# Tonanguyxiro/FastBN

Hardware: AMD Instinct MI355X
Metric: JT test-cases/sec (ALARM, Munin) + PC-stable CI-tests/sec, 1/2/4/8 GPU (higher is better)
Workload: dtype f64

## Files before the change

fastbn_amd/api.py:

```python
import atexit
import ctypes as C
import weakref
import os

import numpy as np

_HERE = os.path.dirname(os.path.abspath(__file__))
LIB_PATH = os.environ.get("FBN_LIB_PATH") or os.path.join(_HERE, "libfastbn.so")

_vp, _i32, _i64, _dbl, _cstr = C.c_void_p, C.c_int32, C.c_int64, C.c_double, C.c_char_p
_pp = C.POINTER(C.c_void_p)

_SIGS = {
    "fbn_version": [_vp, _vp],
    "fbn_device_count": [_vp],
    "fbn_network_load_xmlbif": [_cstr, _pp],
    "fbn_network_create": [C.c_int, _vp, _vp, _vp, _vp, _vp, _pp],
    "fbn_network_node_counts": [_vp, C.c_int, _vp, _vp, _vp, _vp],
    "fbn_network_num_nodes": [_vp, _vp],
    "fbn_network_dims": [_vp, _vp],
    "fbn_network_name": [_vp, C.c_int, C.c_char_p, C.c_int],
    "fbn_network_destroy": [_vp],
    "fbn_evidence_load_libsvm": [_cstr, C.c_int, _vp, _vp, _i64, _vp],
    "fbn_dataset_load_csv": [_cstr, _pp],
# ... 6 lines not shown
    "fbn_dataset_columns": [_vp, _vp],
    "fbn_dataset_var_name": [_vp, C.c_int, C.c_char_p, C.c_int],
    "fbn_dataset_destroy": [_vp],
    "fbn_jt_plan_create": [_vp, C.c_int, _pp],
    "fbn_jt_plan_info_get": [_vp, _vp],
    "fbn_jt_plan_dump": [_vp, _cstr, _cstr],
    "fbn_jt_run": [_vp, _vp, _i64, _vp, _vp, _vp],
    "fbn_jt_run_device": [_vp, _vp, _i64, _vp, _vp, _vp],
    "fbn_jt_evidence_validate": [_vp, _vp, _i64, _vp],
    "fbn_jt_set_evidence_check": [_vp, C.c_int],
    "fbn_jt_set_kernel_timing": [_vp, C.c_int],
    "fbn_jt_score": [_vp, _vp, _vp, _i64, _vp, _vp],
    "fbn_jt_set_output_layout": [_vp, C.c_int],
    "fbn_jt_score_terms_device": [_vp, _vp, _vp, _i64, _vp, _vp],
    "fbn_jt_last_kernel_ms": [_vp, _vp],
    "fbn_jt_stream_schedule": [_vp, _vp, C.c_int64, _vp, C.c_int64, _vp, _vp],
    "fbn_jt_set_waves_per_cu": [_vp, C.c_int],
    "fbn_jt_set_variant": [_vp, C.c_int],
    "fbn_jt_debug_op_cycles": [_vp, C.c_int, _vp],
    "fbn_jt_kernel_source": [_vp, C.c_char_p, C.c_int64, _vp],
    "fbn_jt_kernel_cache_path": [_vp, C.c_char_p, C.c_int64],
    "fbn_jt_kernel_options": [C.c_char_p, C.c_int64],
    "fbn_jt_kernel_build": [_vp],
    "fbn_jt_debug_force_fixup": [_vp, C.c_int],
    "fbn_jt_debug_flagged_blocks": [_vp, _vp],
    "fbn_jt_set_exact": [_vp, C.c_int],
    "fbn_jt_plan_destroy": [_vp],
    "fbn_ci_dataset_upload": [_vp, C.c_int, _i64, _vp, C.c_int, _pp],
    "fbn_ci_dataset_from_device": [_vp, C.c_int, _i64, _vp, C.c_int, _pp],
    "fbn_ci_set_kernel_timing": [_vp, C.c_int],
    "fbn_ci_run": [_vp, _vp, _i64, C.c_int, _dbl, _vp, _vp, _vp, _vp, _vp],
    "fbn_ci_counts": [_vp, C.c_int, C.c_int, _vp, C.c_int, _vp, _i64, _vp],
    "fbn_ci_last_kernel_ms": [_vp, _vp],
    "fbn_ci_decision_margin": [_vp, _vp, _vp, C.c_int],
    "fbn_ci_debug_counts": [_vp, _vp, _i64, C.c_int, _vp, _i64],
    "fbn_pc_decision_margin": [_vp, _vp, _vp],
    "fbn_ci_ctx_destroy": [_vp],
    "fbn_pc_stable": [_vp, _dbl, C.c_int, C.c_int, _pp],
    "fbn_pc_num_levels": [_vp, _vp],
    "fbn_pc_level_tests": [_vp, _vp],
    "fbn_pc_level_launched": [_vp, _vp],
    "fbn_pc_num_edges": [_vp, _vp],
    "fbn_pc_edges": [_vp, _vp],
    "fbn_pc_sepsets": [_vp, _vp, _i64, _vp],
    "fbn_pc_timing": [_vp, _vp, _vp],
    "fbn_pc_path": [_vp, _vp],
# ... 316 lines not shown
        buf = C.create_string_buffer(4096)
        lib.fbn_jt_kernel_cache_path(self._h, buf, 4096)
        return buf.value.decode()

    def debug_force_fixup(self, enable):
        lib.fbn_jt_debug_force_fixup(self._h, int(enable))

    def debug_flagged_blocks(self):
        n = C.c_int64()
        lib.fbn_jt_debug_flagged_blocks(self._h, C.byref(n))
        return n.value

    def set_exact(self, exact):
        lib.fbn_jt_set_exact(self._h, -1 if exact is None else int(bool(exact)))

    def build_kernel(self):
        lib.fbn_jt_kernel_build(self._h)
        return self.kernel_cache_path()

    def refresh_info(self):
        info = _PlanInfo()
        lib.fbn_jt_plan_info_get(self._h, C.byref(info))
        self.info = {k: getattr(info, k) for k, _ in _PlanInfo._fields_}
        return self.info

    def set_variant(self, v):
        lib.fbn_jt_set_variant(self._h, v)

    def infer(self, evidence, marginals=True):
        ev = np.ascontiguousarray(evidence, dtype=np.int8)
        n = ev.shape[0]
        labels = np.zeros(n, np.int32)
        marg = np.zeros((n, self.info["sum_dom"]), np.float64) if marginals else None
        lib.fbn_jt_run(self._h, _p(ev), n, _p(labels), _p(marg), None)
        return labels, marg

    def run_device(self, d_evidence_ptr, ncases, d_labels_ptr, d_marg_ptr, stream_ptr=None):
        lib.fbn_jt_run_device(self._h, d_evidence_ptr, ncases, d_labels_ptr, d_marg_ptr, stream_ptr)

    def validate_device(self, d_evidence_ptr, ncases, stream_ptr=None):
        lib.fbn_jt_evidence_validate(self._h, d_evidence_ptr, ncases, stream_ptr)

    def set_kernel_timing(self, enable):
        lib.fbn_jt_set_kernel_timing(self._h, int(bool(enable)))

    def set_evidence_check(self, enable):
# ... 389 lines not shown
```

fastbn_amd/csrc/capi.hip:

```cpp
#include <hip/hip_runtime.h>
#include <hipcub/hipcub.hpp>
#include <rocblas/rocblas.h>
#include <dlfcn.h>
#include <chrono>

#include <algorithm>
#include <cmath>
#include <cstdio>
#include <cstring>
#include <functional>
#include <memory>
#include <new>
#include <string>

#include "fbn_internal.h"
#include "sample_model.h"
#include "pc_internal.h"
#include "ci_chisq.h"
#include "pc_small.h"
#include "param_counts.h"

extern "C" hipError_t fbn_jt_launch(const JtOp *ops, int nops, const int32_t *aux, const double *initv,
                                    const uint64_t *dig, const int8_t *evid, int V, long long ncases, int SD,
                                    double *marg, int32_t *labels, double *ws, int32_t *wsi, long long NE, int nc,
// ... 764 lines not shown
    int rc = fbn::GenerateJTKernel(p->host, src, &we, iv, nullptr, JtFast(p), p->out_layout == 1);
    if (rc) return rc;
    if (len) *len = (int64_t)src.size() + 1;
    if (buf && cap > 0) {
        const size_t n = std::min<size_t>((size_t)cap - 1, src.size());
        memcpy(buf, src.data(), n);
        buf[n] = 0;
    }
    return FBN_OK;
}

int fbn_jt_kernel_cache_path(const fbn_jt_plan *p, char *buf, int64_t cap) {
    if (!p || !buf || cap <= 0) return SetError(FBN_ERR_ARG, "bad argument");
    if (!p->gen_eligible) return SetError(FBN_ERR_ARG, "plan not eligible for codegen");
    std::string src;
    std::vector<double> iv;
    int64_t we = 0;
    int rc = fbn::GenerateJTKernel(p->host, src, &we, iv, nullptr, JtFast(p), p->out_layout == 1);
    if (rc) return rc;
    snprintf(buf, (size_t)cap, "%s", fbn::JitCachePath(src).c_str());
    return FBN_OK;
}

int fbn_jt_set_exact(fbn_jt_plan *p, int exact) {
    if (!p || exact < -1 || exact > 1) return SetError(FBN_ERR_ARG, "exact must be -1 (auto), 0 (fast) or 1 (exact)");
    p->exact = exact;
    return FBN_OK;
}

int fbn_jt_debug_force_fixup(fbn_jt_plan *p, int enable) {
    if (!p) return SetError(FBN_ERR_ARG, "null pointer");
    p->force_fixup = enable != 0;
    return FBN_OK;
}

int fbn_jt_debug_flagged_blocks(fbn_jt_plan *p, int64_t *count) {
    if (!p || !count) return SetError(FBN_ERR_ARG, "null pointer");
    *count = 0;
    if (p->last_nblk <= 0 || !p->flags.p) return FBN_OK;
    std::vector<int> h((size_t)p->last_nblk);
    FBN_HIP(hipDeviceSynchronize());
    FBN_HIP(hipMemcpy(h.data(), p->flags.p, h.size() * 4, hipMemcpyDeviceToHost));
    for (int f : h) *count += f != 0;
    return FBN_OK;
}

// ... 2035 lines not shown
```

fastbn_amd/csrc/fbn_internal.h:

```cpp
#ifndef FBN_INTERNAL_H
#define FBN_INTERNAL_H

#include <cstdint>
#include <map>
#include <set>
#include <string>
#include <vector>

#include "../../include/fastbn.h"
#include "jt_program.h"

namespace fbn {

int SetError(int code, const char *fmt, ...);

struct Network {
    std::vector<std::string> names;
    std::vector<int> dom;
    std::vector<std::vector<int>> given;
    std::vector<std::vector<int>> parents_asc;
    std::vector<std::vector<int64_t>> counts;
    std::vector<std::vector<int64_t>> totals;
    int n() const { return (int)dom.size(); }
    double Prob(int v, int q, const int *parent_vals_asc) const;
// ... 81 lines not shown
    int64_t store_rows = 0;
    int64_t scratch_row = 0;
    int64_t scratch_rows = 0;
    int num_cliques = 0;
    int sum_dom = 0;
};
int CompileJTProgramV(const JTPlanHost &plan, JTProgramV &prog);

struct JTProgramT {
    std::vector<JtTPass> passes;
    std::vector<int32_t> tab;
    std::vector<double> initv;
    int64_t scr_row = 0;
    int64_t red_row = 0;
    int64_t store_rows = 0;
    int64_t lds_bytes = 0;
    int64_t entry_visits = 0;
    int num_cliques = 0, sum_dom = 0;
    int waves = 1;
};
int CompileJTProgramT(const JTPlanHost &plan, JTProgramT &prog, int lds_budget);

bool JTCodegenEligible(const JTPlanHost &plan, int64_t *entry_ops);
int GenerateJTKernel(const JTPlanHost &plan, std::string &src, int64_t *wave_entries, std::vector<double> &initv,
                     int64_t *lds_bytes = nullptr, bool fast = false, bool var_major = false);

}

struct fbn_network {
    fbn::Network net;
};
struct fbn_dataset {
    fbn::Dataset ds;
};

#endif
```

fastbn_amd/csrc/jt_codegen.cpp:

```cpp
#include <algorithm>
#include <map>
#include <cstdio>
#include <cstdlib>
#include <functional>
#include <sstream>
#include <string>

#include "fbn_internal.h"

namespace fbn {

namespace {

int LocOfT(const Table &t, int v) {
    for (size_t i = 0; i < t.vars.size(); ++i)
        if (t.vars[i] == v) return (int)i;
    return -1;
}

std::string Lit(double x) {
    char b[64];
    snprintf(b, sizeof b, "%.17g", x);
    std::string s = b;
    if (s.find_first_of(".eEn") == std::string::npos) s += ".0";
// ... 4 lines not shown

bool JTCodegenEligible(const JTPlanHost &plan, int64_t *entry_ops) {
    int64_t tmax = 0, ops = 0;
    for (const auto &t : plan.cliques) {
        tmax = std::max<int64_t>(tmax, t.size());
        ops += t.size() * (4 + (int64_t)t.vars.size());
    }
    if (entry_ops) *entry_ops = ops;
    for (int d : plan.dom)
        if (d > 32) return false;
    return tmax <= 256 && ops <= 40000;
}

namespace {

constexpr int kDefaultMerge = 1;

class JTGen {
  public:
    JTGen(const JTPlanHost &p, bool fast_order, bool var_major) : plan(p), fast(fast_order), vmajor(var_major) {}
    int Run(std::string &src, int64_t *wave_entries, std::vector<double> &initv);
    int64_t lds_rows = 0;
    int64_t pool_rows = 0;
    bool iv_lds = false;

  private:
    const JTPlanHost &plan;
    const bool fast;
    const bool vmajor;
    std::ostringstream o;
    std::vector<int> okw_word, okw_pos, out_off;
    std::vector<int64_t> sep_row, init_off;
    std::vector<std::vector<int>> cand;
    std::vector<int> home;
    std::vector<int> msep;
    std::vector<int> mclq;
    void ChooseMarginalSources(const std::vector<int> &pre);
    void MargTerms(int v, const std::vector<std::vector<std::string>> &terms);
    int nobs = 0;
    bool profile = false;
    int merge = 0;
    int64_t init_batch = 16;
    bool in_merged = false;
    int min_waves = 1;
    bool marg_v2 = true, marg_pair = true;
    std::vector<std::vector<std::string>> col_loc, dis_loc;
    std::vector<bool> md_reg;
    std::vector<bool> leaf_rc, col_store;
    void LoadCol(const std::string &name, int s) {
        if (!leaf_rc[s]) return Load(name, s);
        const int c = plan.sep_down[s];
        const int64_t Ts = plan.seps[s].size(), Q = plan.cliques[c].size() / Ts;
        for (int64_t j = 0; j < Ts; ++j) o << "        double " << name << s << "_" << j << ";\n";
        o << "        { // recompute the Collect message of leaf clique " << c << "\n";
        const std::string P = "r" + name;
        InitProd(P, c, {}, -1, "");
        for (int64_t j = 0; j < Ts; ++j) {
            std::vector<std::string> terms;
            for (int64_t q = 0; q < Q; ++q) terms.push_back(N(P, c, q * Ts + j));
            o << "        " << name << s << "_" << j << " = " << TreeSum(terms) << ";\n";
        }
        o << "        }\n";
    }
    void PlaceMessages(const std::vector<int> &post, const std::vector<int> &pre, int64_t budget);
    std::string B(int k) const {
        return profile ? "        FBN_OP_BOUNDARY(); FBN_STAMP(" + std::to_string(k) + ");\n" : "        FBN_OP_BOUNDARY();\n";
    }

    std::string R(int c) const {
        std::vector<unsigned> m(nobs, 0u);
        for (int v : plan.cliques[c].vars) m[v / 32] |= 1u << (v % 32);
        std::ostringstream t;
        t << "(" << plan.cliques[c].vars.size();
        for (int k = 0; k < nobs; ++k)
            if (m[k]) t << " - __builtin_popcount(obs" << k << " & " << m[k] << "u)";
        t << ")";
        return t.str();
    }
    std::string observed(int v) const {
        std::ostringstream t;
        t << "((obs" << v / 32 << " >> " << v % 32 << ") & 1u)";
        return t.str();
    }
    int child(int s) const { return plan.sep_down[s]; }
    int64_t SepIndex(const Table &t, const Table &sp, int64_t e) const {
        int64_t r = e, idx = 0;
        for (size_t j = 0; j < t.vars.size(); ++j) {
// ... 352 lines not shown

void JTGen::ChooseMarginalSources(const std::vector<int> &pre) {
    const int mode = getenv("FBN_JT_MARG_SRC") ? atoi(getenv("FBN_JT_MARG_SRC")) : 0;
    if (mode == 0 || getenv("FBN_JT_NO_SEPMARG")) return;
    const int nc = (int)plan.cliques.size(), ns = (int)plan.seps.size(), V = (int)plan.dom.size();
    std::vector<int> pi(nc);
    for (int k = 0; k < nc; ++k) pi[pre[k]] = k;
    for (int v = 0; v < V; ++v) {
        int best_t = -1, bc = -1, bs = -1;
        int64_t best_sz = 0;
        auto consider = [&](int t, int64_t sz, int c, int sp) {
            const bool better = best_t < 0 || (mode == 1 ? t > best_t : t < best_t) || (t == best_t && sz < best_sz);
            if (better) best_t = t, best_sz = sz, bc = c, bs = sp;
        };
        for (int c : cand[v]) consider(pi[c], plan.cliques[c].size(), c, -1);
        for (int sp = 0; sp < ns; ++sp)
            for (int u : plan.seps[sp].vars)
                if (u == v) consider(pi[plan.sep_up[sp]], plan.seps[sp].size(), -1, sp);
        if (bs >= 0) msep[v] = bs;
        else msep[v] = -1, mclq[v] = bc;
    }
}

void JTGen::PlaceMessages(const std::vector<int> &post, const std::vector<int> &pre, int64_t budget) {
    const int nc = (int)plan.cliques.size(), ns = (int)plan.seps.size();
    auto tsize = [&](int c) { return plan.cliques[c].size(); };
    std::vector<int> pi(nc), qi(nc);
    for (int k = 0; k < nc; ++k) qi[post[k]] = k, pi[pre[k]] = k;
    md_reg.assign(ns, false);
    for (int c : pre)
        if (!plan.clique_down[c].empty()) {
            const int q = pre[pi[c] + 1], s = plan.clique_up[q];
            int64_t mk = 0;
            for (int s2 : plan.clique_down[q]) mk = std::max<int64_t>(mk, plan.seps[s2].size());
            md_reg[s] = tsize(q) + plan.seps[s].size() + mk <= budget;
        }
    const bool no_leaf_rc = !getenv("FBN_JT_LEAF_RC") || atoi(getenv("FBN_JT_LEAF_RC")) == 0;
    leaf_rc.assign(ns, false);
    col_store.assign(ns, true);
    for (int s = 0; s < ns; ++s) {
        const int c = plan.sep_down[s], p = plan.sep_up[s];
        if (!fast || no_leaf_rc || !plan.clique_down[c].empty() || tsize(c) > 64) continue;
        leaf_rc[s] = true;
        col_store[s] = !(qi[p] > 0 && post[qi[p] - 1] == c);
    }
    struct Item {
        int s;
        bool dist;
        int a, b;
        int64_t n;
    };
    std::vector<Item> items;
    for (int s = 0; s < ns; ++s) {
        const int c = plan.sep_down[s], p = plan.sep_up[s];
        if (!leaf_rc[s]) items.push_back({s, false, qi[c], nc + pi[p], plan.seps[s].size()});
        else if (col_store[s]) items.push_back({s, false, qi[c], qi[p], plan.seps[s].size()});
        if (!md_reg[s]) items.push_back({s, true, nc + pi[p], nc + pi[c], plan.seps[s].size()});
    }
    const int64_t per_wave = 160 * 1024 / 4 / 8;
    int64_t ivn = 0;
    for (const auto &t : plan.cliques) ivn += t.size();
    int64_t cap = std::max<int64_t>(0, (per_wave - lds_rows * 64 - (iv_lds ? ivn : 0)) / 64);
    if (const char *e = getenv("FBN_JT_LDS_POOL")) cap = std::min<int64_t>(cap, std::max(0, atoi(e)));
    std::vector<int> order(items.size());
    for (size_t i = 0; i < items.size(); ++i) order[i] = (int)i;
    std::stable_sort(order.begin(), order.end(), [&](int x, int y) {
        return items[x].b - items[x].a < items[y].b - items[y].a;
    });
    std::vector<int64_t> use(2 * nc + 1, 0);
    std::vector<bool> in_lds(items.size(), false);
    for (int i : order) {
        const Item &it = items[i];
        if (it.n > cap) continue;
        int64_t mx = 0;
        for (int t = it.a; t <= it.b; ++t) mx = std::max(mx, use[t]);
        if (mx + it.n > cap) continue;
        for (int t = it.a; t <= it.b; ++t) use[t] += it.n;
        in_lds[i] = true;
    }
    std::vector<int> byst;
    for (size_t i = 0; i < items.size(); ++i)
        if (in_lds[i]) byst.push_back((int)i);
    std::stable_sort(byst.begin(), byst.end(), [&](int x, int y) { return items[x].a < items[y].a; });
    std::vector<std::vector<int64_t>> rows_of(items.size());
    std::vector<int64_t> free_rows;
    for (int64_t r = cap - 1; r >= 0; --r) free_rows.push_back(r);
    std::vector<int> active;
    pool_rows = 0;
    for (int i : byst) {
        const Item &it = items[i];
        for (size_t k = 0; k < active.size();) {
            if (items[active[k]].b < it.a) {
                for (int64_t r : rows_of[active[k]]) free_rows.push_back(r);
                std::sort(free_rows.rbegin(), free_rows.rend());
                active.erase(active.begin() + k);
            } else {
                ++k;
            }
        }
        for (int64_t j = 0; j < it.n; ++j) {
            rows_of[i].push_back(free_rows.back());
            pool_rows = std::max<int64_t>(pool_rows, free_rows.back() + 1);
            free_rows.pop_back();
        }
        active.push_back(i);
    }
    col_loc.assign(ns, {});
    dis_loc.assign(ns, {});
    sep_row.assign(ns, -1);
    int64_t grow = 0;
    for (size_t i = 0; i < items.size(); ++i) {
        const Item &it = items[i];
        auto &loc = it.dist ? dis_loc[it.s] : col_loc[it.s];
        loc.assign(it.n, std::string());
        if (in_lds[i]) {
            for (int64_t j = 0; j < it.n; ++j) loc[j] = "LP(" + std::to_string(rows_of[i][j]) + ")";
            continue;
        }
        if (sep_row[it.s] < 0) sep_row[it.s] = grow, grow += it.n;
        for (int64_t j = 0; j < it.n; ++j) loc[j] = "W(" + std::to_string(sep_row[it.s] + j) + "LL)";
    }
    for (int s = 0; s < ns; ++s) {
        if (sep_row[s] < 0) sep_row[s] = 0;
        if (dis_loc[s].empty()) dis_loc[s].assign(plan.seps[s].size(), "0.0");
        if (col_loc[s].empty()) col_loc[s].assign(plan.seps[s].size(), "0.0");
    }
    if (getenv("FBN_JT_PLACE_DEBUG")) {
        int64_t lc = 0, ld = 0, gc = 0, gd = 0, leaf = 0;
        for (size_t i = 0; i < items.size(); ++i)
            (items[i].dist ? (in_lds[i] ? ld : gd) : (in_lds[i] ? lc : gc)) += items[i].n;
        for (int s = 0; s < ns; ++s)
            if (plan.clique_down[plan.sep_down[s]].empty()) leaf += plan.seps[s].size();
        fprintf(stderr, "placement: pool %lld of %lld rows; Collect rows LDS %lld global %lld; Distribute rows LDS %lld "
                        "global %lld (registers: the rest); global rows %lld; leaf-separator rows %lld\n",
                (long long)pool_rows, (long long)cap, (long long)lc, (long long)gc, (long long)ld, (long long)gd,
                (long long)grow, (long long)leaf);
        std::string u;
        for (int t = 0; t <= 2 * nc; ++t) u += std::to_string(use[t]) + (t == nc - 1 ? " | " : " ");
        fprintf(stderr, "pool rows in use by time (Collect | Distribute): %s\n", u.c_str());
        if (fast) {
            std::string m;
            for (int v = 0; v < (int)plan.dom.size(); ++v) {
                const int t = msep[v] >= 0 ? nc + pi[plan.sep_up[msep[v]]] : nc + pi[mclq[v]];
                m += std::to_string(v) + ":" + std::to_string(t) + " ";
            }
            fprintf(stderr, "marginal time per variable: %s\n", m.c_str());
        }
    }
}

int JTGen::Run(std::string &src, int64_t *wave_entries, std::vector<double> &initv) {
    const int nc = (int)plan.cliques.size(), ns = (int)plan.seps.size(), V = plan.num_nodes;
    if (const char *e = getenv("FBN_JT_REG_ENTRIES")) kRegEntries = std::max<int64_t>(1, atoll(e));
    profile = getenv("FBN_JT_PROFILE") && atoi(getenv("FBN_JT_PROFILE")) != 0;
    merge = fast ? (getenv("FBN_JT_MERGE") ? atoi(getenv("FBN_JT_MERGE")) : kDefaultMerge) : 0;
    init_batch = getenv("FBN_JT_INIT_BATCH") ? std::max<int64_t>(1, atoll(getenv("FBN_JT_INIT_BATCH"))) : 16;
    marg_v2 = fast && (!getenv("FBN_JT_MARG_V2") || atoi(getenv("FBN_JT_MARG_V2")) != 0);
    marg_pair = marg_v2 && (!getenv("FBN_JT_MARG_PAIR") || atoi(getenv("FBN_JT_MARG_PAIR")) != 0);
    min_waves = getenv("FBN_JT_MIN_WAVES") ? std::max(1, atoi(getenv("FBN_JT_MIN_WAVES"))) : min_waves;
// ... 5 lines not shown
    for (int c = 0; c < nc; ++c) {
        init_off[c] = (int64_t)initv.size();
        initv.insert(initv.end(), plan.cliques[c].pot.begin(), plan.cliques[c].pot.end());
    }
    int SD = 0;
    out_off.assign(V, 0);
    for (int v = 0; v < V; ++v) out_off[v] = SD, SD += plan.dom[v];
    cand.assign(V, {});
    for (int c = 0; c < nc; ++c)
        for (int v : plan.cliques[c].vars) cand[v].push_back(c);
    home.assign(V, -1);
    for (int v = 0; v < V; ++v)
        for (int q : cand[v])
            if (home[v] < 0 || plan.cliques[q].size() < plan.cliques[home[v]].size()) home[v] = q;
    msep.assign(V, -1);
    if (fast && !getenv("FBN_JT_NO_SEPMARG"))
        for (int sp = 0; sp < ns; ++sp)
            for (int v : plan.seps[sp].vars) {
                const int64_t have = msep[v] >= 0 ? plan.seps[msep[v]].size() : plan.cliques[home[v]].size();
                if (plan.seps[sp].size() < have) msep[v] = sp;
            }
    mclq = home;
    const int child_order = fast && getenv("FBN_JT_CHILD_ORDER") ? atoi(getenv("FBN_JT_CHILD_ORDER")) : 0;
    auto dfs = [&](bool collect, std::vector<int> &post_o, std::vector<int> &pre_o) {
        std::vector<std::vector<int>> kids(nc);
        for (int c = 0; c < nc; ++c) {
            kids[c] = plan.clique_down[c];
            const bool asc = collect && (child_order & 1), desc = !collect && (child_order & 2);
            if (asc || desc)
                std::stable_sort(kids[c].begin(), kids[c].end(), [&](int x, int y) {
                    return asc ? plan.seps[x].size() < plan.seps[y].size() : plan.seps[x].size() > plan.seps[y].size();
                });
        }
        std::vector<std::pair<int, size_t>> st{{plan.root, 0}};
        while (!st.empty()) {
            auto &top = st.back();
            const int c = top.first;
            if (top.second == 0) pre_o.push_back(c);
            if (top.second < kids[c].size()) {
                const int ch = child(kids[c][top.second++]);
                st.push_back({ch, 0});
            } else {
                post_o.push_back(c);
                st.pop_back();
            }
        }
    };
    std::vector<int> post, pre, unused;
    dfs(true, post, unused);
    unused.clear();
    dfs(false, unused, pre);
    if ((int)post.size() != nc) return SetError(FBN_ERR_LIMIT, "codegen: tree traversal covers %zu of %d cliques", post.size(), nc);
    const int64_t kBudget = getenv("FBN_JT_PREFETCH_BUDGET") ? atoll(getenv("FBN_JT_PREFETCH_BUDGET")) : fast ? 260 : 200;
    if (fast) ChooseMarginalSources(pre);
    PlaceMessages(post, pre, kBudget);
    int64_t rows = 0;
    for (int s = 0; s < ns; ++s) rows = std::max<int64_t>(rows, sep_row[s] + plan.seps[s].size());
    *wave_entries = std::max<int64_t>(rows, 1);

    o << "// generated by libfastbn (jt_codegen.cpp): " << nc << " cliques, " << ns << " separators, "
      << (fast ? "fast" : "exact") << " arithmetic order\n";
    o << "#define FBN_V " << V << "\n#define FBN_SD " << SD << "\n#define FBN_WE " << *wave_entries << "LL\n";
    o << "#define FBN_LP_BASE " << lds_rows << "\n";
    o << "#define FBN_IV_BASE " << (lds_rows + pool_rows) * 64 << "\n#define FBN_NIV " << initv.size() << "\n";
    o << "#define FBN_IV_LDS " << (iv_lds ? 1 : 0) << "\n#define FBN_MIN_WAVES " << min_waves << "\n";
    if (const char *e = getenv("FBN_JT_WS_FOLD")) o << "#define FBN_WS_FOLD " << atoi(e) << "\n";
    if (getenv("FBN_JT_NO_OUT") && atoi(getenv("FBN_JT_NO_OUT")) != 0) o << "#define FBN_NO_OUT 1\n";
    if (vmajor) o << "#define FBN_VMAJOR 1\n";
    o << R"FBN(typedef signed char i8;
__device__ __forceinline__ double dv(double x, double den, double y) {  // x / den (Markstein, see jt_kernels.hip)
    const double q = x * y;
    const double r = __builtin_fma(-den, q, x);
    return __builtin_fma(r, y, q);
}
// row r of the per-wave workspace, this lane: uniform row base (SGPRs) + lane byte offset (VGPR)
typedef __attribute__((address_space(1))) double gdouble;
typedef __attribute__((address_space(1))) char gchar;
typedef __attribute__((address_space(4))) const double cdouble;
// ... 95 lines not shown
    int nokw = 0;
    {
        int pos = 32;
        for (int v = 0; v < V; ++v) {
            if (pos + plan.dom[v] > 32) ++nokw, pos = 0;
            okw_word[v] = nokw - 1, okw_pos[v] = pos, pos += plan.dom[v];
        }
    }
    nobs = (V + 31) / 32;
    {
        std::vector<std::string> regs;
        for (int k = 0; k < nokw; ++k) regs.push_back("okw" + std::to_string(k));
        for (int k = 0; k < nobs; ++k) regs.push_back("obs" + std::to_string(k));
        o << "#define FBN_OP_BOUNDARY() do { __asm__ volatile(\"\" : \"+s\"(Wb), \"+v\"(lo), \"+v\"(ltail), \"+v\"(ivl), \"+v\"(bad), \"+s\"(blkl) :: \"memory\");";
        for (size_t i = 0; i < regs.size(); i += 16) {
            o << " __asm__ volatile(\"\" :";
            for (size_t k = i; k < std::min(regs.size(), i + 16); ++k) o << (k > i ? ", " : " ") << "\"+v\"(" << regs[k] << ")";
            o << ");";
        }
        o << " __builtin_amdgcn_sched_barrier(0); } while (0)\n";
    }
    for (int k = 0; k < nokw; ++k) o << "        unsigned okw" << k << " = 0u;\n";
    for (int k = 0; k < nobs; ++k) o << "        unsigned obs" << k << " = 0u;\n";
    for (int v = 0; v < V; ++v) {
        const unsigned full = (plan.dom[v] >= 32) ? 0xFFFFFFFFu : ((1u << plan.dom[v]) - 1u);
        o << "        { const int x = ev[" << v << "]; okw" << okw_word[v] << " |= (x < 0 ? " << full << "u : (1u << x)) << "
          << okw_pos[v] << "; obs" << v / 32 << " |= (x >= 0 ? 1u : 0u) << " << v % 32 << "; }\n";
    }
    o << B(0);

    auto tsize = [&](int c) { return plan.cliques[c].size(); };
    auto collect_loads = [&](size_t k, std::vector<int> &ls) {
        ls.clear();
        const int c = post[k];
        const auto &down = plan.clique_down[c];
        for (size_t i = 0; i < down.size(); ++i)
            if (!(k > 0 && child(down[i]) == post[k - 1])) ls.push_back(down[i]);
    };
    auto rows_of = [&](const std::vector<int> &ls) {
        int64_t r = 0;
        for (int s : ls) r += plan.seps[s].size();
        return r;
    };
    std::vector<bool> loaded_a(ns, false);
    for (size_t k = 0; k < post.size(); ++k) {
        const int c = post[k];
        std::vector<int> mine, next;
        collect_loads(k, mine);
        o << "        // ---- collect clique " << c << " (" << tsize(c) << " entries)\n";
        for (int s : mine)
            if (!loaded_a[s]) Load("la", s), loaded_a[s] = true;
        if (k + 1 < post.size()) {
            collect_loads(k + 1, next);
            int64_t pend = 0;
            for (int s : mine) pend += plan.seps[s].size();
            if (tsize(c) + pend + rows_of(next) <= kBudget)
                for (int s : next)
                    if (!loaded_a[s]) Load("la", s), loaded_a[s] = true;
        }
        if (!in_merged) o << B(1);
        in_merged = false;
        const auto &down = plan.clique_down[c];
        if (fast) {
            std::vector<std::pair<int, std::string>> kids;
            for (int s : down) kids.push_back({s, loaded_a[s] ? "la" : "mc"});
            InitProd("t", c, kids, -1, "");
        } else {
            Init("t", c);
            for (size_t i = 0; i < down.size(); ++i) {
                const int s = down[i];
                Mul("t", c, s, loaded_a[s] ? "la" : "mc");
            }
        }
        in_merged = fast && (merge & 2) && c != plan.root && k + 1 < post.size() && tsize(c) + tsize(post[k + 1]) <= 96;
        if (c != plan.root) SepCol("t", c, plan.clique_up[c], col_store[plan.clique_up[c]]);
    }
    in_merged = false;
    auto kids_rows = [&](int c) {
        int64_t r = 0;
// ... 2 lines not shown
    };
    auto early_lb = [&](int c) {
        const int up = plan.clique_up[c];
        const int64_t held = (c != plan.root) ? plan.seps[up].size() : 0;
        return tsize(c) + kids_rows(c) + held <= kBudget;
    };
    std::vector<bool> loaded_b(ns, false), loaded_d(ns, false);
    for (size_t k = 0; k < pre.size(); ++k) {
        const int c = pre[k];
        const int up = plan.clique_up[c];
        const bool early = early_lb(c);
        o << "        // ---- distribute clique " << c << " (" << tsize(c) << " entries)\n";
        int64_t pend = 0;
        if (early)
            for (int s : plan.clique_down[c]) {
                if (!loaded_b[s]) LoadCol("lb", s), loaded_b[s] = true;
                pend += plan.seps[s].size();
            }
        if (c != plan.root && md_reg[up]) pend += plan.seps[up].size();
        if (k + 1 < pre.size()) {
            const int nx = pre[k + 1], nup = plan.clique_up[nx];
            const bool ld_next = !md_reg[nup] && plan.sep_up[nup] != c;
            const int64_t nrows = (early_lb(nx) ? kids_rows(nx) : 0) + (ld_next ? plan.seps[nup].size() : 0);
            if (tsize(c) + pend + nrows <= kBudget) {
                if (early_lb(nx))
                    for (int s : plan.clique_down[nx])
                        if (!loaded_b[s] && !leaf_rc[s]) Load("lb", s), loaded_b[s] = true;
                if (ld_next && !loaded_d[nup]) Load("ld", nup), loaded_d[nup] = true;
            }
        }
        o << B(1);
        std::string P = "t";
        if (c != plan.root && fast && early) {
            P = "u";
            if (!md_reg[up] && !loaded_d[up]) Load("ld", up), loaded_d[up] = true, o << B(1);
            std::vector<std::pair<int, std::string>> kids;
            for (int s : plan.clique_down[c]) kids.push_back({s, "lb"});
            InitProd(P, c, kids, up, md_reg[up] ? "md" : "ld");
        } else if (c != plan.root) {
            P = "u";
            Init(P, c);
            for (int s : plan.clique_down[c]) {
                if (!early) LoadCol("lb", s), o << B(1);
                Mul(P, c, s, "lb");
            }
            if (!md_reg[up] && !loaded_d[up]) Load("ld", up), loaded_d[up] = true, o << B(1);
            DMul(P, c, up, md_reg[up] ? "md" : "ld");
// ... 8 lines not shown
        Marg(P, c);
        if (in_merged) o << B(8);
        in_merged = false;
    }
    for (int v = 0; v < V && !marg_v2; ++v) {
        o << "        if (ACT && " << observed(v) << ") {";
        for (int d = 0; d < plan.dom[v]; ++d) o << " OUTS(" << out_off[v] + d << ", 0.0);";
        o << " }\n";
    }
    o << R"(        const bool any_bad = __builtin_amdgcn_ballot_w64(bad != 0u) != 0ull;
        if (lane == 0) flags[blk] = any_bad ? 1 : 0;  // every block writes its flag: no clearing pass
    }
    if (prof && lane == 0)
        for (int k = 0; k < 10; ++k) prof[(unsigned long long)blockIdx.x * 16 + k] = pacc[k];
}
)";
    src = o.str();
    return FBN_OK;
}

}

int GenerateJTKernel(const JTPlanHost &plan, std::string &src, int64_t *wave_entries, std::vector<double> &initv,
                     int64_t *lds_bytes, bool fast, bool var_major) {
    JTGen g(plan, fast, var_major);
    int rc = g.Run(src, wave_entries, initv);
    if (lds_bytes) *lds_bytes = ((g.lds_rows + g.pool_rows) * 64 + (g.iv_lds ? (int64_t)initv.size() : 0)) * 8;
    return rc;
}

}
```

fastbn_amd/prebuild.py:

```python
import os
import tempfile

from . import api, synth

REPO = os.path.dirname(os.path.dirname(os.path.abspath(__file__)))
ALARM_XML = os.path.join(REPO, "tests", "golden", "alarm", "alarm.xml")
SYNTH_SMALL = dict(n=60, seed=5, window=6)


def synth_small_xml(dirname):
    path = os.path.join(dirname, "synth60.xml")
    synth.random_network(SYNTH_SMALL["n"], seed=SYNTH_SMALL["seed"], window=SYNTH_SMALL["window"], path=path)
    return path


def prebuild(xml_paths, layouts=(0,)):
    out = []
    for xml in xml_paths:
        jt = api.JunctionTree(api.Network(xml), device=-1)
        if jt.info["specialized_eligible"]:
            for layout in layouts:
                jt.set_output_layout(layout)
                for exact in (None, True):
                    jt.set_exact(exact)
                    out.append(jt.build_kernel())
    return out


def fixture_xmls(dirname):
    import glob
    import gzip
    out = []
    for gz in sorted(glob.glob(os.path.join(REPO, "tests", "golden", "synth_nets", "*.xml.gz"))):
        path = os.path.join(dirname, os.path.basename(gz)[:-3])
        with gzip.open(gz, "rb") as f, open(path, "wb") as g:
            g.write(f.read())
        out.append(path)
    return out


ALARM_TEST_OPTIONS = ({"FBN_JT_LEAF_RC": "1"}, {"FBN_JT_LDS_POOL": "0"}, {"FBN_JT_MARG_V2": "0"})


def prebuild_options(xml, options):
    import subprocess
    import sys
    out = []
    for opt in options:
        env = dict(os.environ, **opt)
        code = ("import sys; sys.path.insert(0, %r); from fastbn_amd import api; "
                "print(api.JunctionTree(api.Network(%r), device=-1).build_kernel())" % (REPO, xml))
        r = subprocess.run([sys.executable, "-c", code], env=env, capture_output=True, text=True, check=True)
        out.append(r.stdout.strip().splitlines()[-1])
    return out


def prebuild_default(clean=True):
    with tempfile.TemporaryDirectory() as d:
        built = prebuild([ALARM_XML], layouts=(0, 1)) + prebuild([synth_small_xml(d)] + fixture_xmls(d))
    built += prebuild_options(ALARM_XML, ALARM_TEST_OPTIONS)
    if clean:
        keep = {os.path.basename(p) for p in built}
        kdir = os.path.join(REPO, "fastbn_amd", "kcache")
        for f in os.listdir(kdir) if os.path.isdir(kdir) else []:
            if f.endswith(".hsaco") and f not in keep:
                os.remove(os.path.join(kdir, f))
    return built
```

include/fastbn.h:

```cpp
#ifndef FASTBN_H
#define FASTBN_H

#include <stdint.h>

#ifdef __cplusplus
extern "C" {
#endif

typedef enum {
    FBN_OK = 0,
    FBN_ERR_ARG = -1,
    FBN_ERR_IO = -2,
    FBN_ERR_HIP = -3,
    FBN_ERR_NOMEM = -4,
    FBN_ERR_NODEV = -5,
    FBN_ERR_LIMIT = -6
} fbn_err_t;

const char *fbn_last_error(void);
int fbn_version(int *major, int *minor);
int fbn_device_count(int *n);

typedef struct fbn_network fbn_network;

// ... 52 lines not shown
int fbn_jt_stream_schedule(const fbn_jt_plan *p, int32_t *order, int64_t order_cap, int32_t *sched,
                           int64_t sched_cap, int64_t *n_order, int64_t *n_sched);
int fbn_jt_run(fbn_jt_plan *p, const int8_t *evidence, int64_t ncases, int32_t *labels_out,
               double *marginals_out, void *hip_stream);
int fbn_jt_run_device(fbn_jt_plan *p, const int8_t *d_evidence, int64_t ncases, int32_t *d_labels,
                      double *d_marginals, void *hip_stream);
int fbn_jt_evidence_validate(fbn_jt_plan *p, const int8_t *d_evidence, int64_t ncases, void *hip_stream);
int fbn_jt_set_evidence_check(fbn_jt_plan *p, int enable);
int fbn_jt_score(const fbn_jt_plan *p, const double *marginals, const double *golden, int64_t ncases,
                 double *mse_sum, double *hd_sum);
int fbn_jt_set_output_layout(fbn_jt_plan *p, int layout);
int fbn_jt_score_terms_device(fbn_jt_plan *p, const double *d_marginals, const double *d_golden, int64_t ncases,
                              double *d_terms, void *hip_stream);
int fbn_jt_last_kernel_ms(const fbn_jt_plan *p, float *ms);
int fbn_jt_set_kernel_timing(fbn_jt_plan *p, int enable);
int fbn_jt_set_waves_per_cu(fbn_jt_plan *p, int waves);
int fbn_jt_set_variant(fbn_jt_plan *p, int variant);
int fbn_jt_set_exact(fbn_jt_plan *p, int exact);
int fbn_jt_debug_op_cycles(fbn_jt_plan *p, int enable, unsigned long long *cycles);
int fbn_jt_kernel_source(const fbn_jt_plan *p, char *buf, int64_t cap, int64_t *len);
int fbn_jt_debug_force_fixup(fbn_jt_plan *p, int enable);
int fbn_jt_debug_flagged_blocks(fbn_jt_plan *p, int64_t *count);
int fbn_jt_kernel_cache_path(const fbn_jt_plan *p, char *buf, int64_t cap);
int fbn_jt_kernel_build(const fbn_jt_plan *p);
int fbn_jt_kernel_options(char *buf, int64_t cap);
int fbn_jt_tile_program(const fbn_jt_plan *p, int32_t *passes, int32_t *tab, double *initv, int64_t *geometry);
int fbn_jt_plan_destroy(fbn_jt_plan *p);

typedef struct fbn_ci_ctx fbn_ci_ctx;

int fbn_ci_dataset_upload(const uint8_t *cols, int nvars, int64_t nsamples, const int32_t *dims,
                          int device, fbn_ci_ctx **out);
int fbn_ci_dataset_from_device(const uint8_t *d_cols, int nvars, int64_t nsamples, const int32_t *dims,
                               int device, fbn_ci_ctx **out);
int fbn_ci_set_kernel_timing(fbn_ci_ctx *c, int enable);
int fbn_ci_run(fbn_ci_ctx *c, const int32_t *items, int64_t n, int d, double alpha, double *g2,
               int32_t *df, double *p, uint8_t *indep, void *hip_stream);
int fbn_ci_counts(fbn_ci_ctx *c, int x, int y, const int32_t *z, int d, int32_t *counts, int64_t cap,
                  int64_t *cells);
int fbn_ci_last_kernel_ms(const fbn_ci_ctx *c, float *ms);
int fbn_ci_debug_counts(fbn_ci_ctx *c, const int32_t *items, int64_t n, int d, int32_t *counts, int64_t cap);
int fbn_ci_decision_margin(fbn_ci_ctx *c, double *min_margin, int64_t *near_alpha, int reset);
int fbn_ci_ctx_destroy(fbn_ci_ctx *c);

typedef struct fbn_pc_result fbn_pc_result;

// ... 73 lines not shown
```

Before: 855.6 million.

## Park separator messages in registers and search child visit order to minimize spills

Adds a register pool to the JT codegen message placement. Separator message rows whose lifetimes fit under a per-step register budget are kept as named double variables instead of LDS pool or global workspace rows. The codegen also tries nine combinations of child visit order for the collect and distribute traversals and keeps the one with the fewest global rows that does not raise peak register need. Prefetch budgets are reduced by the parked rows. The risks are higher VGPR pressure, which can cause spills or lower occupancy, and longer kernel generation time. A placement query API and extra prebuild variants are added.

```diff
diff --git a/fastbn_amd/api.py b/fastbn_amd/api.py
--- a/fastbn_amd/api.py
+++ b/fastbn_amd/api.py
@@ -52,6 +52,7 @@
     "fbn_jt_kernel_cache_path": [_vp, C.c_char_p, C.c_int64],
     "fbn_jt_kernel_options": [C.c_char_p, C.c_int64],
     "fbn_jt_kernel_build": [_vp],
+    "fbn_jt_kernel_placement": [_vp, _vp],
     "fbn_jt_debug_force_fixup": [_vp, C.c_int],
     "fbn_jt_debug_flagged_blocks": [_vp, _vp],
     "fbn_jt_set_exact": [_vp, C.c_int],
@@ -414,6 +415,12 @@
         info = _PlanInfo()
         lib.fbn_jt_plan_info_get(self._h, C.byref(info))
         self.info = {k: getattr(info, k) for k, _ in _PlanInfo._fields_}
+        if self.info["specialized_eligible"]:
+            rows = np.zeros(8, np.int64)
+            lib.fbn_jt_kernel_placement(self._h, _p(rows))
+            names = ("global_collect", "global_distribute", "lds_collect", "lds_distribute", "reg_collect",
+                     "reg_distribute", "workspace", "lds_pool")
+            self.info.update({"place_rows_" + k: int(v) for k, v in zip(names, rows)})
         return self.info
 
     def set_variant(self, v):
diff --git a/fastbn_amd/csrc/capi.hip b/fastbn_amd/csrc/capi.hip
--- a/fastbn_amd/csrc/capi.hip
+++ b/fastbn_amd/csrc/capi.hip
@@ -810,6 +810,21 @@
     return FBN_OK;
 }
 
+int fbn_jt_kernel_placement(const fbn_jt_plan *p, int64_t *rows) {
+    if (!p || !rows) return SetError(FBN_ERR_ARG, "null pointer");
+    if (!p->gen_eligible) return SetError(FBN_ERR_ARG, "plan not eligible for codegen");
+    std::string src;
+    std::vector<double> iv;
+    int64_t we = 0;
+    fbn::JTPlacement pl;
+    int rc = fbn::GenerateJTKernel(p->host, src, &we, iv, nullptr, JtFast(p), p->out_layout == 1, &pl);
+    if (rc) return rc;
+    const int64_t r[8] = {pl.global[0], pl.global[1], pl.lds[0], pl.lds[1],
+                          pl.reg[0], pl.reg[1], pl.workspace_rows, pl.lds_pool_rows};
+    std::copy(r, r + 8, rows);
+    return FBN_OK;
+}
+
 int fbn_jt_set_exact(fbn_jt_plan *p, int exact) {
     if (!p || exact < -1 || exact > 1) return SetError(FBN_ERR_ARG, "exact must be -1 (auto), 0 (fast) or 1 (exact)");
     p->exact = exact;
diff --git a/fastbn_amd/csrc/fbn_internal.h b/fastbn_amd/csrc/fbn_internal.h
--- a/fastbn_amd/csrc/fbn_internal.h
+++ b/fastbn_amd/csrc/fbn_internal.h
@@ -127,8 +127,14 @@
 int CompileJTProgramT(const JTPlanHost &plan, JTProgramT &prog, int lds_budget);
 
 bool JTCodegenEligible(const JTPlanHost &plan, int64_t *entry_ops);
+struct JTPlacement {
+    int64_t global[2] = {0, 0}, lds[2] = {0, 0}, reg[2] = {0, 0};
+    int64_t workspace_rows = 0;
+    int64_t lds_pool_rows = 0;
+};
 int GenerateJTKernel(const JTPlanHost &plan, std::string &src, int64_t *wave_entries, std::vector<double> &initv,
-                     int64_t *lds_bytes = nullptr, bool fast = false, bool var_major = false);
+                     int64_t *lds_bytes = nullptr, bool fast = false, bool var_major = false,
+                     JTPlacement *placement = nullptr);
 
 }
 
diff --git a/fastbn_amd/csrc/jt_codegen.cpp b/fastbn_amd/csrc/jt_codegen.cpp
--- a/fastbn_amd/csrc/jt_codegen.cpp
+++ b/fastbn_amd/csrc/jt_codegen.cpp
@@ -50,6 +50,7 @@
     int Run(std::string &src, int64_t *wave_entries, std::vector<double> &initv);
     int64_t lds_rows = 0;
     int64_t pool_rows = 0;
+    JTPlacement place;
     bool iv_lds = false;
 
   private:
@@ -90,7 +91,12 @@
         }
         o << "        }\n";
     }
-    void PlaceMessages(const std::vector<int> &post, const std::vector<int> &pre, int64_t budget);
+    void PlaceMessages(const std::vector<int> &post, const std::vector<int> &pre, int64_t budget, int64_t reg_cap,
+                       bool quiet);
+    static constexpr int64_t kRegFile = 256, kRegSlackVM = 16, kRegSlackCM = 32, kDefaultRegPool = kRegFile;
+    int64_t peak_need = 0;
+    std::vector<int64_t> reg_extra;
+    std::vector<std::string> reg_names;
     std::string B(int k) const {
         return profile ? "        FBN_OP_BOUNDARY(); FBN_STAMP(" + std::to_string(k) + ");\n" : "        FBN_OP_BOUNDARY();\n";
     }
@@ -489,7 +495,8 @@
     }
 }
 
-void JTGen::PlaceMessages(const std::vector<int> &post, const std::vector<int> &pre, int64_t budget) {
+void JTGen::PlaceMessages(const std::vector<int> &post, const std::vector<int> &pre, int64_t budget, int64_t reg_cap,
+                          bool quiet) {
     const int nc = (int)plan.cliques.size(), ns = (int)plan.seps.size();
     auto tsize = [&](int c) { return plan.cliques[c].size(); };
     std::vector<int> pi(nc), qi(nc);
@@ -524,25 +531,111 @@
         else if (col_store[s]) items.push_back({s, false, qi[c], qi[p], plan.seps[s].size()});
         if (!md_reg[s]) items.push_back({s, true, nc + pi[p], nc + pi[c], plan.seps[s].size()});
     }
+    std::vector<int> order(items.size());
+    for (size_t i = 0; i < items.size(); ++i) order[i] = (int)i;
+    std::stable_sort(order.begin(), order.end(), [&](int x, int y) {
+        return items[x].b - items[x].a < items[y].b - items[y].a;
+    });
+    std::vector<int64_t> nreg(items.size(), 0);
+    reg_extra.assign(2 * nc + 1, 0);
+    if (reg_cap > 0) {
+        auto kids_rows = [&](int c) {
+            int64_t r = 0;
+            for (int s : plan.clique_down[c]) r += plan.seps[s].size();
+            return r;
+        };
+        auto early_lb = [&](int c) {
+            const int64_t held = (c != plan.root) ? plan.seps[plan.clique_up[c]].size() : 0;
+            return tsize(c) + kids_rows(c) + held <= budget;
+        };
+        std::vector<int64_t> need(2 * nc + 1, 0);
+        std::vector<std::vector<int>> touch(2 * nc + 1);
+        for (int k = 0; k < nc; ++k) {
+            const int c = post[k];
+            need[k] = std::min<int64_t>(tsize(c), kRegEntries) + kids_rows(c);
+            int64_t mine = 0;
+            for (int s : plan.clique_down[c]) {
+                touch[k].push_back(2 * s);
+                if (!(k > 0 && child(s) == post[k - 1])) mine += plan.seps[s].size();
+            }
+            if (k + 1 < nc) {
+                const int nx = post[k + 1];
+                int64_t next = 0;
+                for (int s : plan.clique_down[nx])
+                    if (child(s) != c) next += plan.seps[s].size();
+                if (tsize(c) + mine + next <= budget) {
+                    need[k] += next;
+                    for (int s : plan.clique_down[nx])
+                        if (child(s) != c) touch[k].push_back(2 * s);
+                }
+            }
+        }
+        for (int k = 0; k < nc; ++k) {
+            const int c = pre[k], up = plan.clique_up[c], t = nc + k;
+            const bool early = early_lb(c);
+            int64_t kmax = 0, pend = early ? kids_rows(c) : 0;
+            for (int s : plan.clique_down[c]) {
+                kmax = std::max<int64_t>(kmax, plan.seps[s].size());
+                touch[t].push_back(2 * s);
+                if (md_reg[s]) need[t] += plan.seps[s].size();
+            }
+            need[t] += std::min<int64_t>(tsize(c), kRegEntries) + (early ? kids_rows(c) : kmax);
+            if (c != plan.root) {
+                need[t] += plan.seps[up].size();
+                touch[t].push_back(2 * up + 1);
+                if (md_reg[up]) pend += plan.seps[up].size();
+            }
+            if (k + 1 < nc) {
+                const int nx = pre[k + 1], nup = plan.clique_up[nx];
+                const bool ld_next = !md_reg[nup] && plan.sep_up[nup] != c;
+                const int64_t nrows = (early_lb(nx) ? kids_rows(nx) : 0) + (ld_next ? plan.seps[nup].size() : 0);
+                if (tsize(c) + pend + nrows <= budget) {
+                    need[t] += nrows;
+                    if (early_lb(nx))
+                        for (int s : plan.clique_down[nx]) touch[t].push_back(2 * s);
+                    if (ld_next) touch[t].push_back(2 * nup + 1);
+                }
+            }
+        }
+        peak_need = *std::max_element(need.begin(), need.end());
+        const int64_t slack = vmajor ? kRegSlackVM : kRegSlackCM;
+        std::vector<int64_t> live(2 * nc + 1, 0);
+        for (int i : order) {
+            const Item &it = items[i];
+            const int id = 2 * it.s + (it.dist ? 1 : 0);
+            int64_t room = it.n;
+            for (int t = it.a; t <= it.b; ++t) room = std::min(room, reg_cap - live[t]);
+            std::vector<int> pay;
+            for (int t = it.a; t < it.b; ++t)
+                if (t == it.a || std::find(touch[t].begin(), touch[t].end(), id) == touch[t].end()) pay.push_back(t);
+            for (int t : pay) room = std::min(room, kRegFile - slack - need[t] - reg_extra[t]);
+            if (room <= 0) continue;
+            nreg[i] = room;
+            for (int t = it.a; t <= it.b; ++t) live[t] += room;
+            for (int t : pay) reg_extra[t] += room;
+        }
+        if (!quiet && getenv("FBN_JT_PLACE_DEBUG")) {
+            std::string u;
+            for (int t = 0; t < 2 * nc; ++t)
+                u += std::to_string(need[t]) + "+" + std::to_string(reg_extra[t]) + (t == nc - 1 ? " | " : " ");
+            fprintf(stderr, "register rows by time, the op's own + parked (Collect | Distribute): %s\n", u.c_str());
+        }
+    }
     const int64_t per_wave = 160 * 1024 / 4 / 8;
     int64_t ivn = 0;
     for (const auto &t : plan.cliques) ivn += t.size();
     int64_t cap = std::max<int64_t>(0, (per_wave - lds_rows * 64 - (iv_lds ? ivn : 0)) / 64);
     if (const char *e = getenv("FBN_JT_LDS_POOL")) cap = std::min<int64_t>(cap, std::max(0, atoi(e)));
-    std::vector<int> order(items.size());
-    for (size_t i = 0; i < items.size(); ++i) order[i] = (int)i;
-    std::stable_sort(order.begin(), order.end(), [&](int x, int y) {
-        return items[x].b - items[x].a < items[y].b - items[y].a;
-    });
     std::vector<int64_t> use(2 * nc + 1, 0);
     std::vector<bool> in_lds(items.size(), false);
     for (int i : order) {
         const Item &it = items[i];
-        if (it.n > cap) continue;
+        const int64_t n = it.n - nreg[i];
+        if (n == 0 || n > cap) continue;
         int64_t mx = 0;
         for (int t = it.a; t <= it.b; ++t) mx = std::max(mx, use[t]);
-        if (mx + it.n > cap) continue;
-        for (int t = it.a; t <= it.b; ++t) use[t] += it.n;
+        if (mx + n > cap) continue;
+        for (int t = it.a; t <= it.b; ++t) use[t] += n;
         in_lds[i] = true;
     }
     std::vector<int> byst;
@@ -565,7 +658,7 @@
                 ++k;
             }
         }
-        for (int64_t j = 0; j < it.n; ++j) {
+        for (int64_t j = nreg[i]; j < it.n; ++j) {
             rows_of[i].push_back(free_rows.back());
             pool_rows = std::max<int64_t>(pool_rows, free_rows.back() + 1);
             free_rows.pop_back();
@@ -575,33 +668,50 @@
     col_loc.assign(ns, {});
     dis_loc.assign(ns, {});
     sep_row.assign(ns, -1);
+    reg_names.clear();
+    std::vector<int64_t> sep_skip(ns, 0);
+    for (int s = 0; s < ns; ++s) sep_skip[s] = plan.seps[s].size();
+    for (size_t i = 0; i < items.size(); ++i)
+        if (!in_lds[i]) sep_skip[items[i].s] = std::min(sep_skip[items[i].s], nreg[i]);
     int64_t grow = 0;
+    place = JTPlacement();
     for (size_t i = 0; i < items.size(); ++i) {
         const Item &it = items[i];
         auto &loc = it.dist ? dis_loc[it.s] : col_loc[it.s];
         loc.assign(it.n, std::string());
+        for (int64_t j = 0; j < nreg[i]; ++j) {
+            loc[j] = (it.dist ? "rd" : "rc") + std::to_string(it.s) + "_" + std::to_string(j);
+            reg_names.push_back(loc[j]);
+        }
+        place.reg[it.dist] += nreg[i];
         if (in_lds[i]) {
-            for (int64_t j = 0; j < it.n; ++j) loc[j] = "LP(" + std::to_string(rows_of[i][j]) + ")";
+            for (int64_t j = nreg[i]; j < it.n; ++j) loc[j] = "LP(" + std::to_string(rows_of[i][j - nreg[i]]) + ")";
+            place.lds[it.dist] += it.n - nreg[i];
             continue;
         }
-        if (sep_row[it.s] < 0) sep_row[it.s] = grow, grow += it.n;
-        for (int64_t j = 0; j < it.n; ++j) loc[j] = "W(" + std::to_string(sep_row[it.s] + j) + "LL)";
-    }
+        if (nreg[i] == it.n) continue;
+        if (sep_row[it.s] < 0) sep_row[it.s] = grow, grow += it.n - sep_skip[it.s];
+        for (int64_t j = nreg[i]; j < it.n; ++j) loc[j] = "W(" + std::to_string(sep_row[it.s] + j - sep_skip[it.s]) + "LL)";
+        place.global[it.dist] += it.n - nreg[i];
+    }
+    place.workspace_rows = grow;
+    place.lds_pool_rows = pool_rows;
     for (int s = 0; s < ns; ++s) {
         if (sep_row[s] < 0) sep_row[s] = 0;
         if (dis_loc[s].empty()) dis_loc[s].assign(plan.seps[s].size(), "0.0");
         if (col_loc[s].empty()) col_loc[s].assign(plan.seps[s].size(), "0.0");
     }
-    if (getenv("FBN_JT_PLACE_DEBUG")) {
-        int64_t lc = 0, ld = 0, gc = 0, gd = 0, leaf = 0;
-        for (size_t i = 0; i < items.size(); ++i)
-            (items[i].dist ? (in_lds[i] ? ld : gd) : (in_lds[i] ? lc : gc)) += items[i].n;
+    if (!quiet && getenv("FBN_JT_PLACE_DEBUG")) {
+        int64_t leaf = 0;
         for (int s = 0; s < ns; ++s)
             if (plan.clique_down[plan.sep_down[s]].empty()) leaf += plan.seps[s].size();
         fprintf(stderr, "placement: pool %lld of %lld rows; Collect rows LDS %lld global %lld; Distribute rows LDS %lld "
                         "global %lld (registers: the rest); global rows %lld; leaf-separator rows %lld\n",
-                (long long)pool_rows, (long long)cap, (long long)lc, (long long)gc, (long long)ld, (long long)gd,
-                (long long)grow, (long long)leaf);
+                (long long)pool_rows, (long long)cap, (long long)place.lds[0], (long long)place.global[0],
+                (long long)place.lds[1], (long long)place.global[1], (long long)grow, (long long)leaf);
+        if (reg_cap > 0)
+            fprintf(stderr, "register pool (cap %lld rows): Collect rows %lld, Distribute rows %lld\n", (long long)reg_cap,
+                    (long long)place.reg[0], (long long)place.reg[1]);
         std::string u;
         for (int t = 0; t <= 2 * nc; ++t) u += std::to_string(use[t]) + (t == nc - 1 ? " | " : " ");
         fprintf(stderr, "pool rows in use by time (Collect | Distribute): %s\n", u.c_str());
@@ -653,7 +763,16 @@
             }
     mclq = home;
     const int child_order = fast && getenv("FBN_JT_CHILD_ORDER") ? atoi(getenv("FBN_JT_CHILD_ORDER")) : 0;
-    auto dfs = [&](bool collect, std::vector<int> &post_o, std::vector<int> &pre_o) {
+    std::vector<int64_t> weight(nc, 0);
+    {
+        std::function<int64_t(int)> w = [&](int c) {
+            weight[c] = plan.cliques[c].size();
+            for (int s : plan.clique_down[c]) weight[c] += w(child(s));
+            return weight[c];
+        };
+        w(plan.root);
+    }
+    auto dfs = [&](bool collect, int visit, std::vector<int> &post_o, std::vector<int> &pre_o) {
         std::vector<std::vector<int>> kids(nc);
         for (int c = 0; c < nc; ++c) {
             kids[c] = plan.clique_down[c];
@@ -661,6 +780,10 @@
             if (asc || desc)
                 std::stable_sort(kids[c].begin(), kids[c].end(), [&](int x, int y) {
                     return asc ? plan.seps[x].size() < plan.seps[y].size() : plan.seps[x].size() > plan.seps[y].size();
+                });
+            else if (visit)
+                std::stable_sort(kids[c].begin(), kids[c].end(), [&](int x, int y) {
+                    return visit == 1 ? weight[child(x)] > weight[child(y)] : weight[child(x)] < weight[child(y)];
                 });
         }
         std::vector<std::pair<int, size_t>> st{{plan.root, 0}};
@@ -678,13 +801,35 @@
         }
     };
     std::vector<int> post, pre, unused;
-    dfs(true, post, unused);
+    dfs(true, 0, post, unused);
     unused.clear();
-    dfs(false, unused, pre);
+    dfs(false, 0, unused, pre);
     if ((int)post.size() != nc) return SetError(FBN_ERR_LIMIT, "codegen: tree traversal covers %zu of %d cliques", post.size(), nc);
     const int64_t kBudget = getenv("FBN_JT_PREFETCH_BUDGET") ? atoll(getenv("FBN_JT_PREFETCH_BUDGET")) : fast ? 260 : 200;
+    int64_t reg_cap = fast && vmajor ? kDefaultRegPool : 0;
+    if (const char *e = getenv("FBN_JT_REG_POOL")) reg_cap = fast ? std::max(0, atoi(e)) : 0;
+    if (reg_cap > 0 && child_order == 0) {
+        int64_t best = -1, plan_peak = 0;
+        int bvc = 0, bvd = 0;
+        std::vector<int> bpost = post, bpre = pre;
+        for (int vc = 0; vc < 3; ++vc)
+            for (int vd = 0; vd < 3; ++vd) {
+                std::vector<int> po, pr, un;
+                dfs(true, vc, po, un);
+                un.clear();
+                dfs(false, vd, un, pr);
+                PlaceMessages(po, pr, kBudget, reg_cap, true);
+                if (best < 0) plan_peak = peak_need;
+                else if (peak_need > plan_peak) continue;
+                const int64_t g = place.global[0] + place.global[1];
+                if (best < 0 || g < best) best = g, bpost = po, bpre = pr, bvc = vc, bvd = vd;
+            }
+        post = bpost, pre = bpre;
+        if (getenv("FBN_JT_PLACE_DEBUG"))
+            fprintf(stderr, "child order (0 plan, 1 heaviest subtree first, 2 last): Collect %d, Distribute %d\n", bvc, bvd);
+    }
     if (fast) ChooseMarginalSources(pre);
-    PlaceMessages(post, pre, kBudget);
+    PlaceMessages(post, pre, kBudget, reg_cap, false);
     int64_t rows = 0;
     for (int s = 0; s < ns; ++s) rows = std::max<int64_t>(rows, sep_row[s] + plan.seps[s].size());
     *wave_entries = std::max<int64_t>(rows, 1);
@@ -826,6 +971,11 @@
     }
     for (int k = 0; k < nokw; ++k) o << "        unsigned okw" << k << " = 0u;\n";
     for (int k = 0; k < nobs; ++k) o << "        unsigned obs" << k << " = 0u;\n";
+    for (size_t i = 0; i < reg_names.size(); i += 8) {
+        o << "        double";
+        for (size_t k = i; k < std::min(reg_names.size(), i + 8); ++k) o << (k > i ? ", " : " ") << reg_names[k];
+        o << ";\n";
+    }
     for (int v = 0; v < V; ++v) {
         const unsigned full = (plan.dom[v] >= 32) ? 0xFFFFFFFFu : ((1u << plan.dom[v]) - 1u);
         o << "        { const int x = ev[" << v << "]; okw" << okw_word[v] << " |= (x < 0 ? " << full << "u : (1u << x)) << "
@@ -858,7 +1008,7 @@
             collect_loads(k + 1, next);
             int64_t pend = 0;
             for (int s : mine) pend += plan.seps[s].size();
-            if (tsize(c) + pend + rows_of(next) <= kBudget)
+            if (tsize(c) + pend + rows_of(next) + reg_extra[k] <= kBudget)
                 for (int s : next)
                     if (!loaded_a[s]) Load("la", s), loaded_a[s] = true;
         }
@@ -907,7 +1057,7 @@
             const int nx = pre[k + 1], nup = plan.clique_up[nx];
             const bool ld_next = !md_reg[nup] && plan.sep_up[nup] != c;
             const int64_t nrows = (early_lb(nx) ? kids_rows(nx) : 0) + (ld_next ? plan.seps[nup].size() : 0);
-            if (tsize(c) + pend + nrows <= kBudget) {
+            if (tsize(c) + pend + nrows + reg_extra[nc + k] <= kBudget) {
                 if (early_lb(nx))
                     for (int s : plan.clique_down[nx])
                         if (!loaded_b[s] && !leaf_rc[s]) Load("lb", s), loaded_b[s] = true;
@@ -962,9 +1112,10 @@
 }
 
 int GenerateJTKernel(const JTPlanHost &plan, std::string &src, int64_t *wave_entries, std::vector<double> &initv,
-                     int64_t *lds_bytes, bool fast, bool var_major) {
+                     int64_t *lds_bytes, bool fast, bool var_major, JTPlacement *placement) {
     JTGen g(plan, fast, var_major);
     int rc = g.Run(src, wave_entries, initv);
+    if (placement) *placement = g.place;
     if (lds_bytes) *lds_bytes = ((g.lds_rows + g.pool_rows) * 64 + (g.iv_lds ? (int64_t)initv.size() : 0)) * 8;
     return rc;
 }
diff --git a/fastbn_amd/prebuild.py b/fastbn_amd/prebuild.py
--- a/fastbn_amd/prebuild.py
+++ b/fastbn_amd/prebuild.py
@@ -39,17 +39,19 @@
     return out
 
 
-ALARM_TEST_OPTIONS = ({"FBN_JT_LEAF_RC": "1"}, {"FBN_JT_LDS_POOL": "0"}, {"FBN_JT_MARG_V2": "0"})
+ALARM_TEST_OPTIONS = ({"FBN_JT_LEAF_RC": "1"}, {"FBN_JT_LDS_POOL": "0"}, {"FBN_JT_MARG_V2": "0"},
+                      {"FBN_JT_REG_POOL": "0"}, {"FBN_JT_REG_POOL": "256"})
 
 
-def prebuild_options(xml, options):
+def prebuild_options(xml, options, layout=0):
     import subprocess
     import sys
     out = []
     for opt in options:
         env = dict(os.environ, **opt)
         code = ("import sys; sys.path.insert(0, %r); from fastbn_amd import api; "
-                "print(api.JunctionTree(api.Network(%r), device=-1).build_kernel())" % (REPO, xml))
+                "jt = api.JunctionTree(api.Network(%r), device=-1); jt.set_output_layout(%d); "
+                "print(jt.build_kernel())" % (REPO, xml, layout))
         r = subprocess.run([sys.executable, "-c", code], env=env, capture_output=True, text=True, check=True)
         out.append(r.stdout.strip().splitlines()[-1])
     return out
@@ -59,6 +61,7 @@
     with tempfile.TemporaryDirectory() as d:
         built = prebuild([ALARM_XML], layouts=(0, 1)) + prebuild([synth_small_xml(d)] + fixture_xmls(d))
     built += prebuild_options(ALARM_XML, ALARM_TEST_OPTIONS)
+    built += prebuild_options(ALARM_XML, ({"FBN_JT_REG_POOL": "0"}, {"FBN_JT_REG_POOL": "256"}), layout=1)
     if clean:
         keep = {os.path.basename(p) for p in built}
         kdir = os.path.join(REPO, "fastbn_amd", "kcache")
diff --git a/include/fastbn.h b/include/fastbn.h
--- a/include/fastbn.h
+++ b/include/fastbn.h
@@ -98,6 +98,7 @@
 int fbn_jt_debug_force_fixup(fbn_jt_plan *p, int enable);
 int fbn_jt_debug_flagged_blocks(fbn_jt_plan *p, int64_t *count);
 int fbn_jt_kernel_cache_path(const fbn_jt_plan *p, char *buf, int64_t cap);
+int fbn_jt_kernel_placement(const fbn_jt_plan *p, int64_t *rows);
 int fbn_jt_kernel_build(const fbn_jt_plan *p);
 int fbn_jt_kernel_options(char *buf, int64_t cap);
 int fbn_jt_tile_program(const fbn_jt_plan *p, int32_t *passes, int32_t *tab, double *initv, int64_t *geometry);
```

After: 976.1 million, median of 6. 1.14x the previous value.
